# JustKshitijD/genomicsbench_palisade

Measured on AMD Instinct MI355X. Metric: GCUPS (phmm) + Mreads/s (fmi) on 'large' set at 1/2/4/8 MI355X, higher is better.
Workload: dtype f32+f64 (phmm), int64 (fmi), int32/f64 (chain), int32 (bsw); 1 GPU; phmm large: 64 batches, 755118 testcases, 47.634 G cells per step (whole job); all 755118 testcases; 36.0% of rank 0's testcases on the f64 fallback; parallelism=shard1 (strong scaling, no data-path collective)

## Files before the change

genomicsbench_palisade_amd/csrc/phmm.hip:

```cpp
#include <hip/hip_runtime.h>

#include <algorithm>
#include <cmath>
#include <cstdint>
#include <cstdlib>
#include <chrono>
#include <cstring>
#include <functional>
#include <future>
#include <limits>
#include <mutex>
#include <string>
#include <unordered_map>
#include <thread>
#include <type_traits>
#include <vector>

#include "../../include/gb_phmm.h"
#include "gb_common.h"
#include "gb_common_wave.h"

namespace {

constexpr int kWave = 64;
constexpr int kLdsHaplen = 9400;
constexpr int kMaxHaplen = 65535;
constexpr int kBndPad = 72;
constexpr int kRecPad = 16;
constexpr int kQualTab = 128;
constexpr int kStackRows = 2048;
constexpr int kPlanBuckets = 128;
constexpr int kPlanCount = 8, kPlanCursor = kPlanCount + kPlanBuckets, kPlanTotal = kPlanCursor + kPlanBuckets;
constexpr int kCountWords = kPlanTotal + 8;
constexpr int kMaxF64Parts = 8;
constexpr int kM2M = ((127 * 128) >> 1) + 128;

constexpr int kMaxQual = 254;
constexpr double kJacTol = 8.0;
constexpr double kJacStep = 0.0001;
#define GB_JAC_INV_STEP (1.0 / kJacStep)
constexpr int kJacSize = (int)(kJacTol / kJacStep) + 1;

template <typename T>
struct HostTables {
  T ph2pr[kQualTab];
  T one_minus[kQualTab];
  T div3[kQualTab];
  T m2m[kM2M];
  T init_const;
  T log10_init;
};

template <typename T>
static int fast_round(T d) {
  return (d > (T)0.0) ? (int)(d + (T)0.5) : (int)(d - (T)0.5);
}

template <typename T>
static T log10sum(const std::vector<T> &jac, T small, T big) {
  if (small > big) std::swap(small, big);
  T diff = big - small;
  if (diff >= (T)kJacTol) return big;
  int ind = fast_round<T>((T)(diff * (T)GB_JAC_INV_STEP));
  return big + jac[ind];
}

template <typename T>
static void build_tables(HostTables<T> &t) {
  std::vector<T> jac(kJacSize);
  for (int k = 0; k < kJacSize; k++) jac[k] = (T)(log10(1.0 + pow(10.0, -((double)k) * kJacStep)));
  const double inv_ln10 = 1.0 / log(10);
  std::vector<T> m2m_full(((kMaxQual + 1) * (kMaxQual + 2)) >> 1);
  for (int i = 0, off = 0; i <= kMaxQual; off += ++i)
    for (int j = 0; j <= i; j++) {
      double s = log10sum<T>(jac, (T)(-0.1 * i), (T)(-0.1 * j));
      double l = log1p(-std::min(1.0, pow(10, s))) * inv_ln10;
      m2m_full[off + j] = (T)(pow(10, l));
    }
  for (int k = 0; k < kM2M; k++) t.m2m[k] = m2m_full[k];
  for (int x = 0; x < kQualTab; x++) {
    if constexpr (sizeof(T) == 4)
      t.ph2pr[x] = powf(10.f, -((float)x) / 10.f);
    else
      t.ph2pr[x] = pow(10.0, -((double)x) / 10.0);
    t.one_minus[x] = (T)1.0 - t.ph2pr[x];
    t.div3[x] = t.ph2pr[x] / (T)3.0;
  }
  if constexpr (sizeof(T) == 4) {
    t.init_const = ldexpf(1.f, 120);
    t.log10_init = log10f(t.init_const);
  } else {
    t.init_const = ldexp(1.0, 1020);
    t.log10_init = log10(t.init_const);
  }
}

static uint8_t base_code(char ch) {
  switch ((uint8_t)ch) {
    case 'A': return 0;
    case 'C': return 1;
    case 'T': return 2;
    case 'G': return 3;
    case 'N': return 4;
    default: return 0;
  }
}
static uint8_t read_match_mask(uint8_t rc) { return rc == 4 ? 0x1F : (uint8_t)((1u << rc) | 0x10); }

constexpr double kExitGrowthMax = 2.0;
constexpr uint8_t kMayExit = 0x80;
static double exit_growth(const HostTables<float> &t, const uint8_t *rec, int R) {
  const double inf = std::numeric_limits<double>::infinity();
  double G = 1.0;
  for (int k = 0; k + 1 < R; k++) {
    const int qd = rec[3 * R + k] & 127, qc = rec[4 * R + k] & 127;
    const int ni = rec[2 * R + k + 1] & 127, nd = rec[3 * R + k + 1] & 127, nc = rec[4 * R + k + 1] & 127;
    const int mn = std::min(ni, nd), mx = std::max(ni, nd);
    const double nMM = t.m2m[((mx * (mx + 1)) >> 1) + mn], nMX = t.ph2pr[ni];
    const double nGAPM = t.one_minus[nc], nXX = t.ph2pr[nc];
    const double pYY = t.ph2pr[qc], leak = (double)t.ph2pr[qd] * nGAPM;
    if (leak > 0 && pYY >= 1.0) return inf;
    const double gM = nMM + nMX + (leak > 0 ? leak / (1.0 - pYY) : 0.0), gX = nGAPM + nXX;
    const double g = std::max(gM, gX);
    if (g > 1.0) G *= g;
    if (G > 1e30) return inf;
  }
  return G;
}

struct __attribute__((aligned(16))) TcDesc {
  uint32_t read_off;
  uint32_t hap_off;
  uint32_t dims;
  uint32_t out_idx;
};

template <typename T>
struct DevTab {
  const T *ph2pr, *one_minus, *div3, *m2m;
  T init_const;
};

template <typename T>
struct __attribute__((aligned(2 * sizeof(T)))) Brec {
  T z, w;
};

template <int (*F)(int, int)>
__device__ __forceinline__ float dpp(float v, float keep) {
  return __builtin_bit_cast(float, F(__builtin_bit_cast(int, v), __builtin_bit_cast(int, keep)));
}
template <int (*F)(int, int)>
__device__ __forceinline__ double dpp(double v, double keep) {
  long long vb = __builtin_bit_cast(long long, v), kb = __builtin_bit_cast(long long, keep);
  int lo = F((int)(vb & 0xffffffffll), (int)(kb & 0xffffffffll));
  int hi = F((int)(vb >> 32), (int)(kb >> 32));
  return __builtin_bit_cast(double, ((long long)hi << 32) | (unsigned int)lo);
}
template <int (*F)(int, int)>
__device__ __forceinline__ uint32_t dpp(uint32_t v, uint32_t keep) {
  return (uint32_t)F((int)v, (int)keep);
}

__device__ __forceinline__ float select_dist(uint32_t rmask, uint32_t h, float dmatch, float dmis) {
  uint32_t m = (uint32_t)__builtin_amdgcn_sbfe((int)rmask, h, 1);
  uint32_t r = (m & __builtin_bit_cast(uint32_t, dmatch)) | (~m & __builtin_bit_cast(uint32_t, dmis));
  return __builtin_bit_cast(float, r);
}
__device__ __forceinline__ double select_dist(uint32_t rmask, uint32_t h, double dmatch, double dmis) {
  uint32_t m;
  asm("v_bfe_i32 %0, %1, %2, 1" : "=v"(m) : "v"(rmask), "v"(h));
  const uint64_t a = __builtin_bit_cast(uint64_t, dmatch), b = __builtin_bit_cast(uint64_t, dmis);
  const uint32_t lo = (m & (uint32_t)a) | (~m & (uint32_t)b);
  const uint32_t hi = (m & (uint32_t)(a >> 32)) | (~m & (uint32_t)(b >> 32));
  return __builtin_bit_cast(double, ((uint64_t)hi << 32) | lo);
}

__device__ __forceinline__ uint32_t load_code(const uint8_t *p) {
  uint32_t h = *p;
  asm volatile("" : "+v"(h));
  return h;
}

template <typename T>
struct RowParams {
  T pMY, pYY, dmatch, dmis;
  T nMM, nGAPM, nGAPMx, nMX, nXX;
  uint32_t rmask;
};

template <typename T>
struct LaneState {
  T Mp, Yp, zo, wo, zd;
};

template <typename T, bool kSum, bool kWrite>
__device__ __forceinline__ void phmm_step(const Brec<T> &rec, uint32_t h, LaneState<T> &st,
                                          const RowParams<T> &P, T &sumM, T &sumX, Brec<T> *wr, bool last_lane) {
  const T X = dpp<gb::wave_shr1>(st.wo, rec.w);
  const T zdn = dpp<gb::wave_shr1>(st.zo, rec.z);
  const T dist = select_dist(P.rmask, h, P.dmatch, P.dmis);
  const T M = st.zd * dist;
  const T Y = st.Mp * P.pMY + st.Yp * P.pYY;
  st.zo = (M * P.nMM + X * P.nGAPMx) + Y * P.nGAPM;
  st.wo = M * P.nMX + X * P.nXX;
  if constexpr (kSum) {
    sumM = sumM + M;
    sumX = sumX + X;
  }
  if constexpr (kWrite) {
    if (last_lane) {
      Brec<T> b;
      b.z = st.zo;
      b.w = st.wo;
      *wr = b;
    }
  }
  st.zd = zdn;
  st.Mp = M;
  st.Yp = Y;
}

template <typename T, bool kSum, bool kWrite>
__device__ __forceinline__ void phmm_stripe(int steps, LaneState<T> &st, const RowParams<T> &P,
                                            T &sumM, T &sumX, Brec<T> *__restrict__ bnd,
                                            const uint8_t *__restrict__ hcol, int C, int lane,
                                            uint64_t lastmask, T *__restrict__ out) {
  const uint8_t *hl = hcol + 1 - lane;
  const bool last_lane = lane == kWave - 1;
  constexpr int U = 4;
  constexpr int kNoWrite = 60;
  uint64_t pend = lastmask;
  int target = (kSum && pend) ? C + __builtin_ctzll(pend) - 1 : INT_MAX;
  auto single = [&](int tt, auto wr_tag) {
    constexpr bool W = decltype(wr_tag)::value;
    phmm_step<T, kSum, W>(bnd[tt + 1], load_code(hl + tt), st, P, sumM, sumX, bnd + (tt - (kWave - 2)), last_lane);
    if (kSum && tt == target) {
      if (lane == __builtin_ctzll(pend)) *out = sumM + sumX;
      pend &= pend - 1;
      target = pend ? C + __builtin_ctzll(pend) - 1 : INT_MAX;
    }
  };
  int vzero;
  asm volatile("v_mov_b32 %0, 0" : "=v"(vzero));
  Brec<T> *wb = bnd - (kWave - 2) + vzero;
  auto run = [&](int t, int end, auto wr_tag) {
    constexpr bool W = decltype(wr_tag)::value;
    for (; t + U <= end; t += U) {
      if (kSum && target < t + U) {
        for (int u = 0; u < U; u++) single(t + u, wr_tag);
        continue;
      }
      Brec<T> *wr = wb + t;
      const Brec<T> c0 = wr[kWave - 1], c1 = wr[kWave], c2 = wr[kWave + 1], c3 = wr[kWave + 2];
      const uint32_t h0 = load_code(hl + t), h1 = load_code(hl + t + 1);
      const uint32_t h2 = load_code(hl + t + 2), h3 = load_code(hl + t + 3);
      phmm_step<T, kSum, W>(c0, h0, st, P, sumM, sumX, wr, last_lane);
      phmm_step<T, kSum, W>(c1, h1, st, P, sumM, sumX, wr + 1, last_lane);
      phmm_step<T, kSum, W>(c2, h2, st, P, sumM, sumX, wr + 2, last_lane);
      phmm_step<T, kSum, W>(c3, h3, st, P, sumM, sumX, wr + 3, last_lane);
    }
    for (; t < end; t++) single(t, wr_tag);
  };
  if constexpr (kWrite) {
    const int a = min(steps, kNoWrite);
    run(0, a, std::false_type{});
    run(a, steps, std::true_type{});
  } else {
    run(0, steps, std::false_type{});
  }
}

template <typename T>
__device__ __forceinline__ void load_row(const uint8_t *__restrict__ rbase, int R, int row,
                                         const DevTab<T> &tab, T &pMM, T &pGAPM, T &pMX, T &pXX,
                                         T &pMY, T &pYY, T &dmatch, T &dmis, uint32_t &rmask) {
  rmask = rbase[row];
  const int q = rbase[R + row] & 127, qi = rbase[2 * R + row] & 127;
  const int qd = rbase[3 * R + row] & 127, qc = rbase[4 * R + row] & 127;
  const int mn = qi <= qd ? qi : qd, mx = qi <= qd ? qd : qi;
  pMM = tab.m2m[((mx * (mx + 1)) >> 1) + mn];
  pGAPM = tab.one_minus[qc];
  pMX = tab.ph2pr[qi];
  pXX = tab.ph2pr[qc];
  pMY = tab.ph2pr[qd];
  pYY = tab.ph2pr[qc];
  dmatch = tab.one_minus[q];
  dmis = tab.div3[q];
}

struct __attribute__((aligned(16))) Stack {
  uint32_t first;
  uint32_t count;
  uint32_t hap_off;
  uint32_t C;
};
struct __attribute__((aligned(16))) StackEnt {
  int start;
  int R;
  uint32_t read_off, out_idx;
};

constexpr int kRollGroup = 16;

__host__ __device__ inline uint64_t stack_steps(int rows, int C, int sh, bool roll) {
  const int turns = (rows + sh - 1) / sh;
  if (roll && sh == kWave && C >= kWave && C <= kLdsHaplen && turns >= 2) {
    const int P = (C + kRollGroup + 1 + 3) & ~3;
    return (uint64_t)(turns - 1) * (uint64_t)P + (uint64_t)(C + rows - kWave * (turns - 1));
  }
  return (uint64_t)turns * (uint64_t)(C + sh);
}

template <typename T>
__device__ __forceinline__ void setup_row(int rho, bool dead, int r, int R, const uint8_t *__restrict__ rbase,
                                          const DevTab<T> &tab, T init_Y, T z_top, RowParams<T> &P,
                                          LaneState<T> &st);

template <typename T, bool kExit>
__device__ __forceinline__ int phmm_rolled(const int base, const int T_rows, const int na, const int C, const int lane,
                                           const int e_start, const int e_R, const uint32_t e_read,
                                           const uint32_t e_out, const uint8_t *__restrict__ pool,
                                           const DevTab<T> &tab, const T init_Y, Brec<T> *bnd, const uint8_t *hcol,
                                           T *raw_out, unsigned long long *exit_stats) {
  constexpr int G = kRollGroup, NG = kWave / G, U = 4;
  static_assert(G % U == 0 && G <= kRecPad, "lane 63 writes from its switch on, at columns >= -(G - 1)");
  const int Pd = (C + G + 1 + 3) & ~3;
  const int nturn = (T_rows - base + kWave - 1) / kWave;
  const int t_end = (nturn - 1) * Pd + C + (T_rows - base - kWave * (nturn - 1));
  const bool last_lane = lane == kWave - 1;
  struct L63 {
    int r, R, start, out, may;
  };
  auto setup = [&](int s, RowParams<T> &Q, LaneState<T> &q, L63 &L) {
    const int g = base + kWave * s + lane;
    int lo = 0, hi = na - 1;
    while (__builtin_amdgcn_ballot_w64(lo < hi)) {
      const int mid = (lo + hi + 1) >> 1;
      const int sm = __shfl(e_start, mid);
      if (lo < hi) {
        if (sm <= g) lo = mid; else hi = mid - 1;
      }
    }
    const int start = __shfl(e_start, lo), R = __shfl(e_R, lo);
    const uint32_t roff = (uint32_t)__shfl((int)e_read, lo);
    const int r = g - start;
    setup_row<T>(1, g >= T_rows, r, R, pool + roff, tab, init_Y, (T)0, Q, q);
    if constexpr (kExit) {
      L.r = __builtin_amdgcn_readlane(r, 63);
      L.R = __builtin_amdgcn_readlane(R, 63);
      L.start = __builtin_amdgcn_readlane(start, 63);
      L.out = __builtin_amdgcn_readlane(__shfl((int)e_out, lo), 63);
      L.may = __builtin_amdgcn_readlane((int)Q.rmask, 63) & kMayExit;
    }
  };
  auto uni = [](int v) { return __builtin_amdgcn_readfirstlane(v); };
  RowParams<T> P, Pn;
  LaneState<T> st, sn;
  L63 c63 = {0, 0, 0, 0, 0}, n63 = {0, 0, 0, 0, 0};
  setup(0, P, st, c63);
  setup(1, Pn, sn, n63);
  T sumM = (T)0, sumX = (T)0;
  const uint8_t *hl = hcol - lane;
  constexpr int kFirst = kWave - kRecPad;
  Brec<T> *pp = last_lane ? bnd + (C + kBndPad - kFirst) : bnd;
  int first_t = kFirst;
  int s3 = 0;
  int sw = 0;
  int sw_t = Pd;
  int chk_s = 0;
  int chk_t = kExit ? (kWave + C + 3) & ~3 : INT_MAX;
  struct Target {
    int t, from, lane;
    uint32_t out;
  };
  auto target_of = [&](int en) -> Target {
    const int ec = min(en, na - 1);
    const int d = __builtin_amdgcn_readlane(e_start, ec) + __builtin_amdgcn_readlane(e_R, ec) + 1 - base;
    const int s = d / kWave, l = d % kWave;
    Target g;
    g.lane = l;
    g.t = uni(en < na ? s * Pd + l + C : INT_MAX);
    g.from = uni(en < na ? (s ? s * Pd + (l / G) * G : 0) : INT_MAX);
    g.out = (uint32_t)__builtin_amdgcn_readlane((int)e_out, ec);
    return g;
  };
  int ent = uni((int)__builtin_ctzll(__builtin_amdgcn_ballot_w64(lane < na && e_start + e_R + 1 >= base) | (1ull << 63)));
  Target tg = target_of(ent);
  for (int t = 0; t < t_end;) {
    if constexpr (kExit) {
      if (t == chk_t) {
        if (c63.r >= 2 && c63.r <= c63.R && c63.may) {
          __syncthreads();
          T acc = (T)0;
#pragma unroll 1
          for (int c = 1 + lane; c <= C; c += kWave) acc += bnd[c].z + bnd[c].w;
          for (int o = 32; o >= 1; o >>= 1) acc += __shfl_xor(acc, o);
          if (__builtin_amdgcn_readfirstlane(acc < (T)0.25e-28f ? 1 : 0)) {
            const int next = c63.start + c63.R + 2;
            if (lane == 0) {
              raw_out[(uint32_t)c63.out] = (T)0;
              atomicAdd(exit_stats, 1ull);
              atomicAdd(exit_stats + 1,
                        (unsigned long long)(next - (base + kWave * (chk_s + 1))) * (unsigned long long)C);
            }
            return next;
          }
        }
        chk_s = uni(chk_s + 1);
        chk_t = uni(chk_s + 1 < nturn ? chk_t + Pd : INT_MAX);
      }
    }
    if (t == first_t) {
      if (last_lane) pp = bnd - (kWave - 1);
      first_t = INT_MAX;
    }
    if (t == sw_t) {
      const bool mine = lane / G == sw;
      auto take = [mine](T &cur, T nxt) { cur = mine ? nxt : cur; };
      take(P.pMY, Pn.pMY);
      take(P.pYY, Pn.pYY);
      take(P.dmatch, Pn.dmatch);
      take(P.dmis, Pn.dmis);
      take(P.nMM, Pn.nMM);
      take(P.nGAPM, Pn.nGAPM);
      take(P.nGAPMx, Pn.nGAPMx);
      take(P.nMX, Pn.nMX);
      take(P.nXX, Pn.nXX);
      P.rmask = mine ? Pn.rmask : P.rmask;
      take(st.Mp, (T)0);
      take(st.wo, (T)0);
      take(st.Yp, sn.Yp);
      take(st.zo, sn.zo);
      take(st.zd, sn.zd);
      take(sumM, (T)0);
      take(sumX, (T)0);
      hl -= mine ? Pd : 0;
      if (sw == 0) pp -= last_lane ? 0 : Pd;
      if (sw == NG - 1) {
        s3 = uni(s3 + 1);
        if (last_lane) pp = bnd - (kWave - 1) - s3 * Pd;
        c63 = n63;
        setup(s3 + 1, Pn, sn, n63);
        sw = 0;
        sw_t = uni(s3 + 1 < nturn ? (s3 + 1) * Pd : INT_MAX);
      } else {
        sw = uni(sw + 1);
        sw_t = uni(sw_t + G);
      }
    }
    const bool sum = t >= tg.from;
    int stop = min(min(min(chk_t, sw_t), first_t), min(t_end & ~(U - 1), tg.t & ~(U - 1)));
    if (!sum) stop = min(stop, tg.from);
    stop = uni(stop);
    if (t < stop) {
      auto run = [&](auto sum_tag) {
        constexpr bool S = decltype(sum_tag)::value;
        do {
          Brec<T> *wp = pp + t;
          const uint8_t *hp = hl + t;
          const Brec<T> c0 = wp[0], c1 = wp[1], c2 = wp[2], c3 = wp[3];
          const uint32_t h0 = load_code(hp), h1 = load_code(hp + 1), h2 = load_code(hp + 2), h3 = load_code(hp + 3);
          phmm_step<T, S, true>(c0, h0, st, P, sumM, sumX, wp, last_lane);
          phmm_step<T, S, true>(c1, h1, st, P, sumM, sumX, wp + 1, last_lane);
          phmm_step<T, S, true>(c2, h2, st, P, sumM, sumX, wp + 2, last_lane);
          phmm_step<T, S, true>(c3, h3, st, P, sumM, sumX, wp + 3, last_lane);
          t += U;
        } while (t < stop);
      };
      if (sum) run(std::true_type{}); else run(std::false_type{});
    } else {
      const int n = min(U, t_end - t);
      Brec<T> *wp = pp + t;
      const uint8_t *hp = hl + t;
#pragma unroll 1
      for (int u = 0; u < n; u++) {
        const Brec<T> c = wp[u];
        const uint32_t h = load_code(hp + u);
        phmm_step<T, true, true>(c, h, st, P, sumM, sumX, wp + u, last_lane);
        if (t + u == tg.t) {
          if (lane == tg.lane) raw_out[tg.out] = sumM + sumX;
          ent = uni(ent + 1);
          tg = target_of(ent);
        }
      }
      t += n;
    }
  }
  return T_rows;
}

template <typename T, bool kF64Pass, bool kExit = false, bool kRoll = false>
__device__ __forceinline__ int phmm_stack(const Stack &S, const uint32_t *__restrict__ stk_tc, const TcDesc *__restrict__ descs,
                          const uint8_t *__restrict__ pool, const DevTab<T> &tab, T *__restrict__ raw_out,
                          const float *__restrict__ raw_f, bool force, uint8_t *smem_raw, int part = 0,
                          int parts = 1, unsigned long long *exit_stats = nullptr, bool roll = false) {
  const int lane = threadIdx.x;
  const int C = (int)S.C;
  Brec<T> *bnd = reinterpret_cast<Brec<T> *>(smem_raw) + kRecPad;
  uint8_t *hcol = smem_raw + sizeof(Brec<T>) * (size_t)(C + kBndPad + kRecPad) + kWave;

  TcDesc d = {0, 0, 0, 0};
  bool act = lane < (int)S.count;
  if (parts > 1) act = act && lane >= part * (int)S.count / parts && lane < (part + 1) * (int)S.count / parts;
  if (act) {
    d = descs[stk_tc[S.first + lane]];
    if constexpr (kF64Pass) act = force || raw_f[d.out_idx] < 1e-28f;
  }
  const uint64_t am = __builtin_amdgcn_ballot_w64(act);
  if (!am) return 0;
  const int na = __builtin_popcountll(am);
  const int rows = act ? (int)(d.dims & 0xffff) + 2 : 0;
  const int incl = gb::scan_add(rows);
  const int T_rows = __builtin_amdgcn_readlane(incl, 63);
  int src = 0;
  {
    uint64_t m = am;
    for (int a = 0; a < lane && m; a++) m &= m - 1;
    src = m ? __builtin_ctzll(m) : 63;
  }
  const int e_start = __shfl(incl - rows, src), e_R = __shfl(rows - 2, src);
  const uint32_t e_read = (uint32_t)__shfl((int)d.read_off, src), e_out = (uint32_t)__shfl((int)d.out_idx, src);
  const T init_Y = tab.init_const / (T)C;
  const uint8_t *hcode = pool + S.hap_off;
  for (int c = lane; c < C + kBndPad; c += kWave) {
    Brec<T> b;
    b.z = (T)0;
    b.w = (T)0;
    bnd[c] = b;
  }
  for (int c = lane - kWave; c < C + kBndPad; c += kWave)
    hcol[c] = (c >= 1 && c <= C) ? hcode[c - 1] : (c == 0 ? 5 : (c < 0 ? 6 : 0));
  __syncthreads();

  for (int base = 0; base < T_rows;) {
    if constexpr (kRoll) {
      if (roll && C >= kWave && T_rows - base > kWave) {
        base = phmm_rolled<T, kExit && !kF64Pass>(base, T_rows, na, C, lane, e_start, e_R, e_read, e_out, pool, tab,
                                                  init_Y, bnd, hcol, raw_out, exit_stats);
        __syncthreads();
        continue;
      }
    }
    const int g = base + lane;
    int lo = 0, hi = na - 1;
    while (__builtin_amdgcn_ballot_w64(lo < hi)) {
      const int mid = (lo + hi + 1) >> 1;
      const int sm = __shfl(e_start, mid);
      if (lo < hi) {
        if (sm <= g) lo = mid; else hi = mid - 1;
      }
    }
    StackEnt e;
    e.start = __shfl(e_start, lo);
    e.R = __shfl(e_R, lo);
    e.read_off = (uint32_t)__shfl((int)e_read, lo);
    e.out_idx = (uint32_t)__shfl((int)e_out, lo);
    const int r = g - e.start;
    const bool dead = g >= T_rows;
    const uint8_t *rbase = pool + e.read_off;
    RowParams<T> P;
    LaneState<T> st;
    st.Mp = st.zo = st.wo = (T)0;
    st.Yp = (T)0;
    st.zd = lane == 0 ? bnd[0].z : (T)0;
    {
      T pMM, pGAPM, pMX, pXX, a, b, dm, dx;
      uint32_t f;
      const T zero = (T)0, one = (T)1;
      P.nMM = P.nGAPM = P.nGAPMx = P.nMX = P.nXX = zero;
      if (dead) {
        P.pMY = P.pYY = P.dmatch = P.dmis = zero;
        P.rmask = 0;
      } else if (r == 0) {
        P.pMY = zero;
        P.pYY = one;
        P.dmatch = P.dmis = zero;
        P.rmask = 0;
        P.nGAPM = one;
        st.Yp = init_Y;
        st.zo = (zero * zero + zero * zero) + init_Y * one;
      } else if (r == 1) {
        P.pMY = P.pYY = zero;
        P.dmatch = one;
        P.dmis = zero;
        P.rmask = 0x3F;
        load_row(rbase, e.R, 0, tab, pMM, pGAPM, pMX, pXX, a, b, dm, dx, f);
        P.nMM = pGAPM;
        st.zd = init_Y;
        if (lane == 0) st.zo = (init_Y * P.nMM + zero * zero) + zero * zero;
      } else {
        load_row(rbase, e.R, r - 2, tab, pMM, pGAPM, pMX, pXX, P.pMY, P.pYY, P.dmatch, P.dmis, P.rmask);
        if (r - 1 < e.R) {
          load_row(rbase, e.R, r - 1, tab, P.nMM, P.nGAPM, P.nMX, P.nXX, a, b, dm, dx, f);
          P.nGAPMx = P.nGAPM;
        }
      }
    }
    const bool last_row = !dead && r == e.R + 1;
    const uint64_t lastmask = __builtin_amdgcn_ballot_w64(last_row);
    const bool more = base + kWave < T_rows;
    const int steps = more ? C + kWave - 1 : C + (T_rows - base) - 1;
    T sumM = (T)0, sumX = (T)0;
    T *out = raw_out + e.out_idx;
    int r63 = 0, R63 = 0, start63 = 0, out63 = 0;
    if (kExit && more) {
      r63 = __builtin_amdgcn_readlane(r, 63);
      R63 = __builtin_amdgcn_readlane(e.R, 63);
      start63 = __builtin_amdgcn_readlane(e.start, 63);
      out63 = __builtin_amdgcn_readlane((int)e.out_idx, 63);
    }
    if (lastmask) {
      if (more)
        phmm_stripe<T, true, true>(steps, st, P, sumM, sumX, bnd, hcol, C, lane, lastmask, out);
      else
        phmm_stripe<T, true, false>(steps, st, P, sumM, sumX, bnd, hcol, C, lane, lastmask, out);
    } else {
      phmm_stripe<T, false, true>(steps, st, P, sumM, sumX, bnd, hcol, C, lane, 0, out);
    }
    __syncthreads();
    int next = base + kWave;
    if constexpr (!kF64Pass && kExit) {
      if (r63 >= 2 && r63 <= R63 && (__builtin_amdgcn_readlane((int)P.rmask, 63) & kMayExit)) {
        T acc = (T)0;
#pragma unroll 1
        for (int c = 1 + lane; c <= C; c += kWave) acc += bnd[c].z + bnd[c].w;
        for (int o = 32; o >= 1; o >>= 1) acc += __shfl_xor(acc, o);
        if (__builtin_amdgcn_readfirstlane(acc < (T)0.25e-28f ? 1 : 0)) {
          next = start63 + R63 + 2;
          if (lane == 0) {
            raw_out[(uint32_t)out63] = (T)0;
            atomicAdd(exit_stats, 1ull);
            atomicAdd(exit_stats + 1, (unsigned long long)(next - (base + kWave)) * (unsigned long long)C);
          }
        }
        __syncthreads();
      }
    }
    base = next;
  }
  return na;
}

constexpr int kRows2 = 2 * kWave;
constexpr int kBndPad2 = 136;
constexpr int kCodePad2 = kRows2;
constexpr int kNoWrite2 = kRows2 - 4;

template <typename T>
__device__ __forceinline__ void setup_row(int rho, bool dead, int r, int R, const uint8_t *__restrict__ rbase,
                                          const DevTab<T> &tab, T init_Y, T z_top, RowParams<T> &P,
                                          LaneState<T> &st) {
  st.Mp = st.zo = st.wo = (T)0;
  st.Yp = (T)0;
  st.zd = rho == 0 ? z_top : (T)0;
  T pMM, pGAPM, pMX, pXX, a, b, dm, dx;
  uint32_t f;
  const T zero = (T)0, one = (T)1;
  P.nMM = P.nGAPM = P.nGAPMx = P.nMX = P.nXX = zero;
  if (dead) {
    P.pMY = P.pYY = P.dmatch = P.dmis = zero;
    P.rmask = 0;
  } else if (r == 0) {
    P.pMY = zero;
    P.pYY = one;
    P.dmatch = P.dmis = zero;
    P.rmask = 0;
    P.nGAPM = one;
    st.Yp = init_Y;
    st.zo = (zero * zero + zero * zero) + init_Y * one;
  } else if (r == 1) {
    P.pMY = P.pYY = zero;
    P.dmatch = one;
    P.dmis = zero;
    P.rmask = 0x3F;
    load_row(rbase, R, 0, tab, pMM, pGAPM, pMX, pXX, a, b, dm, dx, f);
    P.nMM = pGAPM;
    st.zd = init_Y;
    if (rho == 0) st.zo = (init_Y * P.nMM + zero * zero) + zero * zero;
  } else {
    load_row(rbase, R, r - 2, tab, pMM, pGAPM, pMX, pXX, P.pMY, P.pYY, P.dmatch, P.dmis, P.rmask);
    if (r - 1 < R) {
      load_row(rbase, R, r - 1, tab, P.nMM, P.nGAPM, P.nMX, P.nXX, a, b, dm, dx, f);
      P.nGAPMx = P.nGAPM;
    }
  }
}

template <typename T, bool kSum, bool kWrite>
__device__ __forceinline__ void phmm_step2(const Brec<T> &rec, uint32_t h, uint32_t &hb, LaneState<T> &A,
                                           LaneState<T> &B, const RowParams<T> &PA, const RowParams<T> &PB,
                                           T &sMa, T &sXa, T &sMb, T &sXb, Brec<T> *wr, bool last_lane) {
  const T Xb = A.wo;
  const T zdnb = A.zo;
  const T Xa = dpp<gb::wave_shr1>(B.wo, rec.w);
  const T zdna = dpp<gb::wave_shr1>(B.zo, rec.z);
  const T Mb = B.zd * select_dist(PB.rmask, hb, PB.dmatch, PB.dmis);
  const T Ma = A.zd * select_dist(PA.rmask, h, PA.dmatch, PA.dmis);
  const T Yb = B.Mp * PB.pMY + B.Yp * PB.pYY;
  const T Ya = A.Mp * PA.pMY + A.Yp * PA.pYY;
  B.zo = (Mb * PB.nMM + Xb * PB.nGAPMx) + Yb * PB.nGAPM;
  B.wo = Mb * PB.nMX + Xb * PB.nXX;
  A.zo = (Ma * PA.nMM + Xa * PA.nGAPMx) + Ya * PA.nGAPM;
  A.wo = Ma * PA.nMX + Xa * PA.nXX;
  if constexpr (kSum) {
    sMa = sMa + Ma;
    sXa = sXa + Xa;
    sMb = sMb + Mb;
    sXb = sXb + Xb;
  }
  if constexpr (kWrite) {
    if (last_lane) {
      Brec<T> r;
      r.z = B.zo;
      r.w = B.wo;
      *wr = r;
    }
  }
  A.zd = zdna;
  A.Mp = Ma;
  A.Yp = Ya;
  B.zd = zdnb;
  B.Mp = Mb;
  B.Yp = Yb;
  hb = h;
}

template <typename T, bool kSum, bool kWrite>
__device__ __forceinline__ void phmm_stripe2(int steps, LaneState<T> &A, LaneState<T> &B, const RowParams<T> &PA,
                                             const RowParams<T> &PB, Brec<T> *__restrict__ bnd,
                                             const uint8_t *__restrict__ hcol, int C, int lane, uint64_t pa,
                                             uint64_t pb, T *__restrict__ outA, T *__restrict__ outB) {
  const uint8_t *hl = hcol + 1 - 2 * lane;
  const bool last_lane = lane == kWave - 1;
  constexpr int U = 4;
  T sMa = (T)0, sXa = (T)0, sMb = (T)0, sXb = (T)0;
  uint32_t hb = hl[-1];
  auto next_target = [&]() -> int {
    if (!kSum || !(pa | pb)) return INT_MAX;
    const int ra = pa ? 2 * __builtin_ctzll(pa) : INT_MAX / 2;
    const int rb = pb ? 2 * __builtin_ctzll(pb) + 1 : INT_MAX / 2;
    return C + min(ra, rb) - 1;
  };
  int target = next_target();
  auto single = [&](int tt, auto wr_tag) {
    constexpr bool W = decltype(wr_tag)::value;
    phmm_step2<T, kSum, W>(bnd[tt + 1], hl[tt], hb, A, B, PA, PB, sMa, sXa, sMb, sXb, bnd + (tt - (kRows2 - 2)),
                           last_lane);
    if (kSum && tt == target) {
      const int rho = tt - C + 1;
      if (rho & 1) {
        if (lane == (rho >> 1)) *outB = sMb + sXb;
        pb &= pb - 1;
      } else {
        if (lane == (rho >> 1)) *outA = sMa + sXa;
        pa &= pa - 1;
      }
      target = next_target();
    }
  };
  int vzero;
  asm volatile("v_mov_b32 %0, 0" : "=v"(vzero));
  Brec<T> *wb = bnd - (kRows2 - 2) + vzero;
  auto run = [&](int t, int end, auto wr_tag) {
    constexpr bool W = decltype(wr_tag)::value;
    for (; t + U <= end; t += U) {
      if (kSum && target < t + U) {
        for (int u = 0; u < U; u++) single(t + u, wr_tag);
        continue;
      }
      Brec<T> *wr = wb + t;
      const Brec<T> c0 = wr[kRows2 - 1], c1 = wr[kRows2], c2 = wr[kRows2 + 1], c3 = wr[kRows2 + 2];
      const uint32_t h0 = hl[t], h1 = hl[t + 1], h2 = hl[t + 2], h3 = hl[t + 3];
      phmm_step2<T, kSum, W>(c0, h0, hb, A, B, PA, PB, sMa, sXa, sMb, sXb, wr, last_lane);
      phmm_step2<T, kSum, W>(c1, h1, hb, A, B, PA, PB, sMa, sXa, sMb, sXb, wr + 1, last_lane);
      phmm_step2<T, kSum, W>(c2, h2, hb, A, B, PA, PB, sMa, sXa, sMb, sXb, wr + 2, last_lane);
      phmm_step2<T, kSum, W>(c3, h3, hb, A, B, PA, PB, sMa, sXa, sMb, sXb, wr + 3, last_lane);
    }
    for (; t < end; t++) single(t, wr_tag);
  };
  if constexpr (kWrite) {
    const int a = min(steps, kNoWrite2);
    run(0, a, std::false_type{});
    run(a, steps, std::true_type{});
  } else {
    run(0, steps, std::false_type{});
  }
}

template <typename T>
__device__ __forceinline__ void phmm_stack2(const Stack &S, const uint32_t *__restrict__ stk_tc,
                                            const TcDesc *__restrict__ descs, const uint8_t *__restrict__ pool,
                                            const DevTab<T> &tab, T *__restrict__ raw_out, uint8_t *smem_raw) {
  const int lane = threadIdx.x;
  const int C = (int)S.C;
  Brec<T> *bnd = reinterpret_cast<Brec<T> *>(smem_raw) + kRecPad;
  uint8_t *hcol = smem_raw + sizeof(Brec<T>) * (size_t)(C + kBndPad2 + kRecPad) + kCodePad2;
  const int na = (int)S.count;
  TcDesc d = {0, 0, 0, 0};
  if (lane < na) d = descs[stk_tc[S.first + lane]];
  const int rows = lane < na ? (int)(d.dims & 0xffff) + 2 : 0;
  const int incl = gb::scan_add(rows);
  const int T_rows = __builtin_amdgcn_readlane(incl, 63);
  const int e_start = incl - rows, e_R = rows - 2;
  const T init_Y = tab.init_const / (T)C;
  const uint8_t *hcode = pool + S.hap_off;
  for (int c = lane; c < C + kBndPad2; c += kWave) {
    Brec<T> b;
    b.z = (T)0;
    b.w = (T)0;
    bnd[c] = b;
  }
  for (int c = lane - kCodePad2; c < C + kBndPad2; c += kWave)
    hcol[c] = (c >= 1 && c <= C) ? hcode[c - 1] : (c == 0 ? 5 : (c < 0 ? 6 : 0));
  __syncthreads();

  const int nstripes = (T_rows + kRows2 - 1) / kRows2;
  for (int s = 0; s < nstripes; s++) {
    const int g0 = s * kRows2 + 2 * lane, g1 = g0 + 1;
    int lo = 0, hi = na - 1;
    while (__builtin_amdgcn_ballot_w64(lo < hi)) {
      const int mid = (lo + hi + 1) >> 1;
      const int sm = __shfl(e_start, mid);
      if (lo < hi) {
        if (sm <= g0) lo = mid; else hi = mid - 1;
      }
    }
    const int nxt = __shfl(e_start, min(lo + 1, kWave - 1));
    const int lob = (lo + 1 < na && nxt <= g1) ? lo + 1 : lo;
    const int sa = __shfl(e_start, lo), Ra = __shfl(e_R, lo);
    const uint32_t rda = (uint32_t)__shfl((int)d.read_off, lo), oa = (uint32_t)__shfl((int)d.out_idx, lo);
    const int sb = __shfl(e_start, lob), Rb = __shfl(e_R, lob);
    const uint32_t rdb = (uint32_t)__shfl((int)d.read_off, lob), ob = (uint32_t)__shfl((int)d.out_idx, lob);
    const int ra = g0 - sa, rb = g1 - sb;
    const bool deadA = g0 >= T_rows, deadB = g1 >= T_rows;
    RowParams<T> PA, PB;
    LaneState<T> A, B;
    const T z_top = lane == 0 ? bnd[0].z : (T)0;
    setup_row<T>(2 * lane, deadA, ra, Ra, pool + rda, tab, init_Y, z_top, PA, A);
    setup_row<T>(2 * lane + 1, deadB, rb, Rb, pool + rdb, tab, init_Y, (T)0, PB, B);
    const uint64_t pa = __builtin_amdgcn_ballot_w64(!deadA && ra == Ra + 1);
    const uint64_t pb = __builtin_amdgcn_ballot_w64(!deadB && rb == Rb + 1);
    const bool more = s < nstripes - 1;
    const int steps = more ? C + kRows2 - 1 : C + (T_rows - s * kRows2) - 1;
    T *outA = raw_out + oa, *outB = raw_out + ob;
    if (pa | pb) {
      if (more)
        phmm_stripe2<T, true, true>(steps, A, B, PA, PB, bnd, hcol, C, lane, pa, pb, outA, outB);
      else
        phmm_stripe2<T, true, false>(steps, A, B, PA, PB, bnd, hcol, C, lane, pa, pb, outA, outB);
    } else {
      phmm_stripe2<T, false, true>(steps, A, B, PA, PB, bnd, hcol, C, lane, 0, 0, outA, outB);
    }
    __syncthreads();
  }
}

template <int W>
__global__ __launch_bounds__(64) __attribute__((amdgpu_waves_per_eu(W ? W : 1, 8))) void phmm_forward2(
                                                     const Stack *__restrict__ stacks,
                                                     const uint32_t *__restrict__ stk_tc,
                                                     const TcDesc *__restrict__ descs,
                                                     const uint8_t *__restrict__ pool, DevTab<float> tab,
                                                     float *__restrict__ raw_out) {
  extern __shared__ __attribute__((aligned(16))) uint8_t smem_raw[];
  phmm_stack2<float>(stacks[blockIdx.x], stk_tc, descs, pool, tab, raw_out, smem_raw);
}

template <typename T, bool kF64Pass, bool kLong = false, bool kExit = false>
__global__ __launch_bounds__(64) __attribute__((amdgpu_waves_per_eu(kLong ? 1 : (sizeof(T) == 4 ? 8 : 4), 8))) void phmm_forward(
    const Stack *__restrict__ stacks, int nstacks,
                                                    const uint32_t *__restrict__ stk_tc,
                                                    const TcDesc *__restrict__ descs,
                                                    const uint8_t *__restrict__ pool, DevTab<T> tab,
                                                    T *__restrict__ raw_out, const float *__restrict__ raw_f,
                                                    int *__restrict__ counter, int force, uint8_t *scratch,
                                                    size_t scratch_stride, const uint32_t *__restrict__ units) {
  extern __shared__ __attribute__((aligned(16))) uint8_t smem_raw[];
  uint8_t *rec = kLong ? scratch + (size_t)blockIdx.x * scratch_stride : smem_raw;
  const bool roll = (force >> 16) & 1;
  if constexpr (kF64Pass || kLong) {
    int done = 0;
    int *next = counter + (kLong ? (kF64Pass ? 3 : 2) : 1);
    const int parts = (kF64Pass && !kLong) ? max(1, (force >> 8) & 0xFF) : 1;
    const int nwork = units ? __builtin_amdgcn_readfirstlane(counter[kPlanTotal]) : nstacks * parts;
    while (true) {
      int k = 0;
      if (threadIdx.x == 0) k = atomicAdd(next, 1);
      k = __builtin_amdgcn_readfirstlane(__shfl(k, 0));
      if (k >= nwork) break;
      if (units) k = __builtin_amdgcn_readfirstlane((int)units[k]);
      done += phmm_stack<T, kF64Pass, false, !kLong>(stacks[k / parts], stk_tc, descs, pool, tab, raw_out, raw_f,
                                                     (force & 0xFF) != 0, rec, k % parts, parts, nullptr, roll);
      __syncthreads();
    }
    if (kF64Pass && threadIdx.x == 0 && done) atomicAdd(counter, done);
  } else {
    phmm_stack<T, false, kExit, true>(stacks[blockIdx.x], stk_tc, descs, pool, tab, raw_out, nullptr, false, rec, 0, 1,
                                      reinterpret_cast<unsigned long long *>(counter + 4), roll);
  }
}

__global__ __launch_bounds__(256) void f64_plan(const Stack *__restrict__ stacks, int nunits, int parts,
                                                const uint32_t *__restrict__ stk_tc, const TcDesc *__restrict__ descs,
                                                const float *__restrict__ raw_f, int force, int roll,
                                                uint8_t *__restrict__ ukey, int *__restrict__ counter) {
  __shared__ int hist[kPlanBuckets];
  for (int i = threadIdx.x; i < kPlanBuckets; i += blockDim.x) hist[i] = 0;
  __syncthreads();
  const int u = blockIdx.x * blockDim.x + threadIdx.x;
  if (u < nunits) {
    const Stack S = stacks[u / parts];
    const int part = u % parts, lo = part * (int)S.count / parts, hi = (part + 1) * (int)S.count / parts;
    int rows = 0;
    for (int a = lo; a < hi; a++) {
      const TcDesc d = descs[stk_tc[S.first + a]];
      if (force || raw_f[d.out_idx] < 1e-28f) rows += (int)(d.dims & 0xffff) + 2;
    }
    int key = 0;
    if (rows) {
      key = (int)((stack_steps(rows, (int)S.C, kWave, roll != 0) + 63) / 64);
      key = key < 1 ? 1 : (key > kPlanBuckets - 1 ? kPlanBuckets - 1 : key);
      atomicAdd(&hist[key], 1);
    }
    ukey[u] = (uint8_t)key;
  }
  __syncthreads();
  for (int i = threadIdx.x; i < kPlanBuckets; i += blockDim.x)
    if (hist[i]) atomicAdd(&counter[kPlanCount + i], hist[i]);
}
// ... 971 lines not shown
```

Before: 1589 GCUPS (phmm).

## Pack next-row params into compact descriptors and expand at switch time

The rolled pHMM kernel no longer keeps a full second copy of RowParams and LaneState for the upcoming row. It stores a two-word packed descriptor (quality codes, flags, m2m index) and expands it into table lookups only when a lane group switches rows, which is meant to cut VGPR pressure and raise occupancy. The lane-63 early-exit info is now recomputed with a ballot instead of being carried along. The wave reduction uses ds_swizzle xor steps instead of shfl_xor. The trade-off is extra table loads and ALU work at each group switch.

```diff
diff --git a/genomicsbench_palisade_amd/csrc/phmm.hip b/genomicsbench_palisade_amd/csrc/phmm.hip
--- a/genomicsbench_palisade_amd/csrc/phmm.hip
+++ b/genomicsbench_palisade_amd/csrc/phmm.hip
@@ -174,6 +174,33 @@
   const uint32_t lo = (m & (uint32_t)a) | (~m & (uint32_t)b);
   const uint32_t hi = (m & (uint32_t)(a >> 32)) | (~m & (uint32_t)(b >> 32));
   return __builtin_bit_cast(double, ((uint64_t)hi << 32) | lo);
+}
+
+template <int O>
+__device__ __forceinline__ float swz_xor(float v) {
+  return __builtin_bit_cast(float, __builtin_amdgcn_ds_swizzle(__builtin_bit_cast(int, v), (O << 10) | 0x1F));
+}
+template <int O>
+__device__ __forceinline__ double swz_xor(double v) {
+  const long long b = __builtin_bit_cast(long long, v);
+  const int lo = __builtin_amdgcn_ds_swizzle((int)(b & 0xffffffffll), (O << 10) | 0x1F);
+  const int hi = __builtin_amdgcn_ds_swizzle((int)(b >> 32), (O << 10) | 0x1F);
+  return __builtin_bit_cast(double, ((long long)hi << 32) | (unsigned int)lo);
+}
+template <typename T>
+__device__ __forceinline__ T wave_sum_xor(T acc) {
+  acc += __shfl_xor(acc, 32);
+  acc += swz_xor<16>(acc);
+  acc += swz_xor<8>(acc);
+  acc += swz_xor<4>(acc);
+  acc += swz_xor<2>(acc);
+  acc += swz_xor<1>(acc);
+  return acc;
+}
+
+__device__ __forceinline__ int fresh(int v) {
+  asm volatile("" : "+v"(v));
+  return v;
 }
 
 __device__ __forceinline__ uint32_t load_code(const uint8_t *p) {
@@ -312,11 +339,6 @@
   return (uint64_t)turns * (uint64_t)(C + sh);
 }
 
-template <typename T>
-__device__ __forceinline__ void setup_row(int rho, bool dead, int r, int R, const uint8_t *__restrict__ rbase,
-                                          const DevTab<T> &tab, T init_Y, T z_top, RowParams<T> &P,
-                                          LaneState<T> &st);
-
 template <typename T, bool kExit>
 __device__ __forceinline__ int phmm_rolled(const int base, const int T_rows, const int na, const int C, const int lane,
                                            const int e_start, const int e_R, const uint32_t e_read,
@@ -332,7 +354,11 @@
   struct L63 {
     int r, R, start, out, may;
   };
-  auto setup = [&](int s, RowParams<T> &Q, LaneState<T> &q, L63 &L) {
+  constexpr uint32_t kReal = 1u << 28, kNext = 1u << 29, kVa = 1u << 30, kV0 = 1u << 31;
+  struct RowDesc {
+    uint32_t own, nxt;
+  };
+  auto describe = [&](int s) -> RowDesc {
     const int g = base + kWave * s + lane;
     int lo = 0, hi = na - 1;
     while (__builtin_amdgcn_ballot_w64(lo < hi)) {
@@ -343,27 +369,72 @@
       }
     }
     const int start = __shfl(e_start, lo), R = __shfl(e_R, lo);
-    const uint32_t roff = (uint32_t)__shfl((int)e_read, lo);
+    const uint8_t *rb = pool + (uint32_t)__shfl((int)e_read, lo);
     const int r = g - start;
-    setup_row<T>(1, g >= T_rows, r, R, pool + roff, tab, init_Y, (T)0, Q, q);
-    if constexpr (kExit) {
-      L.r = __builtin_amdgcn_readlane(r, 63);
-      L.R = __builtin_amdgcn_readlane(R, 63);
-      L.start = __builtin_amdgcn_readlane(start, 63);
-      L.out = __builtin_amdgcn_readlane(__shfl((int)e_out, lo), 63);
-      L.may = __builtin_amdgcn_readlane((int)Q.rmask, 63) & kMayExit;
-    }
+    const bool live = g < T_rows;
+    const bool real = live && r >= 2, below = live && r >= 1 && r <= R;
+    RowDesc D;
+    D.own = (live && r == 1) ? 0x3Fu : 0u;
+    D.nxt = real ? kReal : (live ? (r == 0 ? kVa : kV0) : 0u);
+    if (real) {
+      const uint8_t *p = rb + (r - 2);
+      D.own = (uint32_t)p[0] | (uint32_t)(p[R] & 127) << 8 | (uint32_t)(p[3 * R] & 127) << 16 |
+              (uint32_t)(p[4 * R] & 127) << 24;
+    }
+    if (below) {
+      const uint8_t *p = rb + (r - 1);
+      const uint32_t qi = p[2 * R] & 127, qd = p[3 * R] & 127, qc = p[4 * R] & 127;
+      const uint32_t mn = qi <= qd ? qi : qd, mx = qi <= qd ? qd : qi;
+      D.nxt |= (((mx * (mx + 1)) >> 1) + mn) | qi << 14 | qc << 21 | (real ? kNext : 0u);
+    }
+    return D;
+  };
+  auto expand = [&](const RowDesc &D, bool mine, RowParams<T> &P, LaneState<T> &st) {
+    if (mine) {
+      const T zero = (T)0, one = (T)1;
+      const bool real = D.nxt & kReal, nextr = D.nxt & kNext, va = D.nxt & kVa, v0 = D.nxt & kV0;
+      const uint32_t q = (D.own >> 8) & 127, qd = (D.own >> 16) & 127, qc = D.own >> 24;
+      const uint32_t nqi = (D.nxt >> 14) & 127, nqc = (D.nxt >> 21) & 127;
+      const T tMY = tab.ph2pr[qd], tYY = tab.ph2pr[qc], tdm = tab.one_minus[q], tdx = tab.div3[q];
+      const T tMM = tab.m2m[D.nxt & 0x3FFF], tGAPM = tab.one_minus[nqc], tMX = tab.ph2pr[nqi], tXX = tab.ph2pr[nqc];
+      P.rmask = D.own & 0xFF;
+      P.pMY = real ? tMY : zero;
+      P.pYY = real ? tYY : (va ? one : zero);
+      P.dmatch = real ? tdm : (v0 ? one : zero);
+      P.dmis = real ? tdx : zero;
+      P.nMM = nextr ? tMM : (v0 ? tGAPM : zero);
+      P.nGAPMx = nextr ? tGAPM : zero;
+      P.nGAPM = nextr ? tGAPM : (va ? one : zero);
+      P.nMX = nextr ? tMX : zero;
+      P.nXX = nextr ? tXX : zero;
+      st.Mp = st.wo = zero;
+      st.Yp = st.zo = va ? init_Y : zero;
+      st.zd = v0 ? init_Y : zero;
+    }
+  };
+  auto row63 = [&](int s, const RowParams<T> &P) -> L63 {
+    const int g = base + kWave * s + kWave - 1;
+    const int e = __builtin_popcountll(__builtin_amdgcn_ballot_w64(lane < na && e_start <= g)) - 1;
+    L63 L;
+    L.start = __builtin_amdgcn_readlane(e_start, e);
+    L.R = __builtin_amdgcn_readlane(e_R, e);
+    L.out = __builtin_amdgcn_readlane((int)e_out, e);
+    L.r = g - L.start;
+    L.may = __builtin_amdgcn_readlane((int)P.rmask, 63) & kMayExit;
+    return L;
   };
   auto uni = [](int v) { return __builtin_amdgcn_readfirstlane(v); };
-  RowParams<T> P, Pn;
-  LaneState<T> st, sn;
-  L63 c63 = {0, 0, 0, 0, 0}, n63 = {0, 0, 0, 0, 0};
-  setup(0, P, st, c63);
-  setup(1, Pn, sn, n63);
+  RowParams<T> P;
+  LaneState<T> st;
+  expand(describe(0), true, P, st);
+  L63 c63 = {0, 0, 0, 0, 0};
+  if constexpr (kExit) c63 = row63(0, P);
+  RowDesc nd = describe(1);
   T sumM = (T)0, sumX = (T)0;
-  const uint8_t *hl = hcol - lane;
+  const int ln = fresh(lane);
+  const uint8_t *hl = hcol - ln;
   constexpr int kFirst = kWave - kRecPad;
-  Brec<T> *pp = last_lane ? bnd + (C + kBndPad - kFirst) : bnd;
+  Brec<T> *pp = ln == kWave - 1 ? bnd + (C + kBndPad - kFirst) : bnd;
   int first_t = kFirst;
   int s3 = 0;
   int sw = 0;
@@ -394,8 +465,8 @@
           __syncthreads();
           T acc = (T)0;
 #pragma unroll 1
-          for (int c = 1 + lane; c <= C; c += kWave) acc += bnd[c].z + bnd[c].w;
-          for (int o = 32; o >= 1; o >>= 1) acc += __shfl_xor(acc, o);
+          for (int c = 1 + fresh(lane); c <= C; c += kWave) acc += bnd[c].z + bnd[c].w;
+          acc = wave_sum_xor(acc);
           if (__builtin_amdgcn_readfirstlane(acc < (T)0.25e-28f ? 1 : 0)) {
             const int next = c63.start + c63.R + 2;
             if (lane == 0) {
@@ -417,31 +488,17 @@
     }
     if (t == sw_t) {
       const bool mine = lane / G == sw;
-      auto take = [mine](T &cur, T nxt) { cur = mine ? nxt : cur; };
-      take(P.pMY, Pn.pMY);
-      take(P.pYY, Pn.pYY);
-      take(P.dmatch, Pn.dmatch);
-      take(P.dmis, Pn.dmis);
-      take(P.nMM, Pn.nMM);
-      take(P.nGAPM, Pn.nGAPM);
-      take(P.nGAPMx, Pn.nGAPMx);
-      take(P.nMX, Pn.nMX);
-      take(P.nXX, Pn.nXX);
-      P.rmask = mine ? Pn.rmask : P.rmask;
-      take(st.Mp, (T)0);
-      take(st.wo, (T)0);
-      take(st.Yp, sn.Yp);
-      take(st.zo, sn.zo);
-      take(st.zd, sn.zd);
-      take(sumM, (T)0);
-      take(sumX, (T)0);
-      hl -= mine ? Pd : 0;
-      if (sw == 0) pp -= last_lane ? 0 : Pd;
+      expand(nd, mine, P, st);
+      if (mine) {
+        sumM = sumX = (T)0;
+        hl -= Pd;
+      }
+      if (sw == 0) pp -= last_lane ? 0 : fresh(Pd);
       if (sw == NG - 1) {
         s3 = uni(s3 + 1);
         if (last_lane) pp = bnd - (kWave - 1) - s3 * Pd;
-        c63 = n63;
-        setup(s3 + 1, Pn, sn, n63);
+        if constexpr (kExit) c63 = row63(s3, P);
+        nd = describe(s3 + 1);
         sw = 0;
         sw_t = uni(s3 + 1 < nturn ? (s3 + 1) * Pd : INT_MAX);
       } else {
@@ -624,8 +681,8 @@
       if (r63 >= 2 && r63 <= R63 && (__builtin_amdgcn_readlane((int)P.rmask, 63) & kMayExit)) {
         T acc = (T)0;
 #pragma unroll 1
-        for (int c = 1 + lane; c <= C; c += kWave) acc += bnd[c].z + bnd[c].w;
-        for (int o = 32; o >= 1; o >>= 1) acc += __shfl_xor(acc, o);
+        for (int c = 1 + fresh(lane); c <= C; c += kWave) acc += bnd[c].z + bnd[c].w;
+        acc = wave_sum_xor(acc);
         if (__builtin_amdgcn_readfirstlane(acc < (T)0.25e-28f ? 1 : 0)) {
           next = start63 + R63 + 2;
           if (lane == 0) {
```

Result: faster. 1628 GCUPS (phmm) (median of 6 runs) (+2.5%).
